# ViV99/slam-experiments

Hardware: AMD Instinct MI355X
Metric: descriptor pairs/sec BF-Hamming knn=2 @64kx64k (higher is better)
Workload: dtype u32

## Files before the change

include/slamhip.h:

```cpp
#ifndef SLAMHIP_H
#define SLAMHIP_H

#include <stdint.h>

#ifdef __cplusplus
extern "C" {
#endif

typedef struct slam_ctx slam_ctx;

#define SLAM_API __attribute__((visibility("default")))

enum slam_status {
    SLAM_OK = 0,
    SLAM_ERR_INVALID = -1,
    SLAM_ERR_HIP = -2,
    SLAM_ERR_NO_DEVICE = -3,
    SLAM_ERR_RCCL = -4,
    SLAM_ERR_STATE = -5,
    SLAM_ERR_BUSY = -6
};

#define SLAM_DESC_BYTES 32
#define SLAM_MAX_TRAIN_PER_PASS (1 << 23)
// ... 29 lines not shown
typedef struct slam_bf_search {
    const void* d_query;
    int64_t N;
    const void* d_train;
    int64_t M;
    int64_t train_base;
    int32_t* d_idx;
    int32_t* d_dist;
} slam_bf_search;
SLAM_API int slam_bf_knn2_batch_u256(slam_ctx* ctx, int64_t B, const slam_bf_search* h_searches);

SLAM_API int slam_bf_merge_top2(slam_ctx* ctx, const int32_t* d_idx_parts,
                       const int32_t* d_dist_parts, int64_t G, int64_t N,
                       int32_t* d_idx, int32_t* d_dist);

SLAM_API int slam_bf_knn2_u256_host(slam_ctx* ctx, const uint8_t* h_query, int64_t N,
                           const uint8_t* h_train, int64_t M,
                           int32_t* h_idx, int32_t* h_dist);

#define SLAM_BF_KNN_MAX 32
SLAM_API int slam_bf_knn_u256(slam_ctx* ctx, const void* d_query, int64_t N, const void* d_train, int64_t M,
                              int64_t train_base, int K, int32_t* d_idx, int32_t* d_dist);
SLAM_API int slam_bf_knn_u256_host(slam_ctx* ctx, const uint8_t* h_query, int64_t N, const uint8_t* h_train, int64_t M,
                                   int K, int32_t* h_idx, int32_t* h_dist);
SLAM_API int slam_bf_merge_topk(slam_ctx* ctx, const int32_t* d_idx_parts, const int32_t* d_dist_parts, int64_t G,
                                int64_t N, int K, int32_t* d_idx, int32_t* d_dist);
SLAM_API int slam_bf_topk_plan_describe(int num_cu, int64_t N, int64_t M, int K, int32_t* h_plan);

SLAM_API int slam_bf_radius_u256(slam_ctx* ctx, const void* d_query, int64_t N, const void* d_train, int64_t M,
                                 float max_distance, int64_t train_base, int64_t* d_offsets, int64_t capacity,
                                 int32_t* d_idx, int32_t* d_dist, int64_t* h_total);
SLAM_API int slam_bf_radius_u256_host(slam_ctx* ctx, const uint8_t* h_query, int64_t N, const uint8_t* h_train, int64_t M,
                                      float max_distance, int64_t* h_offsets, int64_t capacity, int32_t* h_idx,
                                      int32_t* h_dist, int64_t* h_total);
SLAM_API int slam_bf_radius_threshold(float max_distance);
SLAM_API int slam_bf_radius_plan_describe(int num_cu, int64_t N, int64_t M, int32_t* h_plan);

SLAM_API int slam_bf_window_knn_u256(slam_ctx* ctx, const void* d_query, int64_t N, const void* d_train, int64_t M,
                                     const float* d_query_xy, const float* d_train_xy, const float* d_radius, float radius,
                                     int k, int64_t cells, int32_t* d_idx, int32_t* d_dist);
SLAM_API int slam_bf_window_knn_u256_host(slam_ctx* ctx, const uint8_t* h_query, int64_t N, const uint8_t* h_train, int64_t M,
                                          const float* h_query_xy, const float* h_train_xy, const float* h_radius,
                                          float radius, int k, int64_t cells, int32_t* h_idx, int32_t* h_dist);
SLAM_API int slam_bf_window_plan_describe(int num_cu, int64_t N, int64_t M, int64_t cells, int64_t* h_plan);

#define SLAM_BF_KNOBS 10
SLAM_API int slam_bf_set_tuning(slam_ctx* ctx, const int32_t* h_knobs, int count);
SLAM_API int slam_bf_plan_info(slam_ctx* ctx, int64_t N, int64_t M, int32_t* h_plan);
SLAM_API int slam_bf_plan_describe(int num_cu, const int32_t* h_knobs, int count, int64_t N, int64_t M, int64_t qb_all,
                                   int rows_on_host, int32_t* h_plan, int32_t* h_tbl, int64_t tbl_cap, int64_t* tbl_len);
SLAM_API int slam_bf_set_engine(slam_ctx* ctx, int engine);
SLAM_API int slam_bf_mx_plan_describe(int num_cu, int64_t N, int64_t M, int32_t* h_plan, int32_t* h_tbl, int64_t tbl_cap,
                                      int64_t* tbl_len);
SLAM_API int slam_bf_reset_state(slam_ctx* ctx);
SLAM_API int slam_bf_state_dirty(slam_ctx* ctx, int64_t* h_words);

SLAM_API int slam_bf_knn2_select_u256(slam_ctx* ctx, const void* d_query, int64_t N, const void* d_train, int64_t M,
                                      int64_t train_base, int32_t* d_idx, int32_t* d_dist, int mode, double param,
                                      uint8_t* d_keep, int64_t* h_count);

SLAM_API int slam_bf_match_filter(slam_ctx* ctx, const int32_t* d_idx, const int32_t* d_dist,
                         int64_t N, int mode, double param,
                         uint8_t* d_keep, int64_t* h_count, int32_t* h_min_dist);

SLAM_API int slam_bf_cross_check(slam_ctx* ctx, const int32_t* d_fwd_idx, const int32_t* d_fwd_dist, int64_t N,
                        const int32_t* d_rev_idx, int64_t M, int32_t* d_out_idx, int32_t* d_out_dist,
                        int64_t* h_count);

SLAM_API int slam_bf_split_index(slam_ctx* ctx, const int32_t* d_global_idx, int64_t count, const int32_t* d_offsets,
                                 int64_t images, int32_t* d_img_idx, int32_t* d_train_idx);

SLAM_API int slam_reproj_rj_f64(slam_ctx* ctx, const double* d_poses, int64_t K,
                       const double* d_points, int64_t L,
                       const int32_t* d_obs_pose, const int32_t* d_obs_point,
                       const double* d_meas, int64_t O,
                       double fx, double fy, double cx, double cy,
                       double* d_e, double* d_Jpose, double* d_Jpoint);

SLAM_API int slam_index_errors(slam_ctx* ctx, int64_t* count);

SLAM_API int slam_pose_normal_eq_f64(slam_ctx* ctx, const double* d_pose,
                            const double* d_points, const double* d_meas,
                            const uint8_t* d_active, int64_t O,
                            double fx, double fy, double cx, double cy,
                            double huber_delta,
                            double* d_H, double* d_b, double* d_chi2);

SLAM_API int slam_pose_optimize_f64(slam_ctx* ctx, const double* d_pose_in, const double* d_points,
                                    const double* d_meas, int64_t O, double fx, double fy, double cx, double cy,
                                    int rounds, int iterations, double chi2_threshold, double huber_delta,
                                    double* d_pose_out, uint8_t* d_inlier, double* d_chi2, int32_t* d_stats);

SLAM_API int slam_pose_optimize_batch_f64(slam_ctx* ctx, int64_t B, const double* d_pose_in, const double* d_points,
                                          const double* d_meas, const int32_t* d_offsets, int64_t O_total, double fx,
                                          double fy, double cx, double cy, int rounds, int iterations,
                                          double chi2_threshold, double huber_delta, double* d_pose_out,
                                          uint8_t* d_inlier, double* d_chi2, int32_t* d_stats);


SLAM_API int slam_tv_fivepoint_f64(slam_ctx* ctx, int64_t S, const double* d_x1, const double* d_x2, double* d_E,
                                   int32_t* d_nroots);

SLAM_API int slam_tv_essential_ransac_f64(slam_ctx* ctx, int64_t B, const int32_t* d_offsets, const double* d_px1,
                                          const double* d_px2, int64_t M, double fx, double fy, double cx, double cy,
                                          int H, double threshold_px, uint64_t seed, double* d_E, uint8_t* d_inlier,
                                          int32_t* d_stats);
// ... 219 lines not shown
```

slam-experiments_amd/csrc/bf_mx.hip:

```cpp
#include "internal.h"
#include <vector>
#include <atomic>
#include <type_traits>

#include "bf_common.h"

#define SLAM_MX_STAGE 128
#define SLAM_MX_BOUND_LIMIT 0x7F000000u
#define SLAM_MX_EARLY 0x16u
#define SLAM_MX_UNROLL 4
#define SLAM_MX_RESIDENT 4

#ifdef SLAM_MX_PROBE
__device__ unsigned long long* g_mx_probe = nullptr;
extern "C" __attribute__((visibility("default"))) int slam_exp_set_mx_probe(void* p) {
    return (int)hipMemcpyToSymbol(HIP_SYMBOL(g_mx_probe), &p, sizeof(p));
}
#define MX_STAMP(ph) do { const unsigned long long now_ = __builtin_readcyclecounter(); pacc[ph] += now_ - plast; plast = now_; } while (0)
#else
#define MX_STAMP(ph) do {} while (0)
#endif

typedef int mx_v8i __attribute__((ext_vector_type(8)));
typedef float mx_v4f __attribute__((ext_vector_type(4)));

__device__ __forceinline__ uint4 mx_expand(u32 x) {
    uint4 r;
    r.x = ((x << 3) & 0x88888888u) | 0x22222222u;
    r.y = ((x << 2) & 0x88888888u) | 0x22222222u;
    r.z = ((x << 1) & 0x88888888u) | 0x22222222u;
    r.w = (x & 0x88888888u) | 0x22222222u;
    return r;
}

__device__ __forceinline__ mx_v4f mx_dot(uint4 a, uint4 b, mx_v4f c) {
    const mx_v8i av = {(int)a.x, (int)a.y, (int)a.z, (int)a.w, 0, 0, 0, 0};
    const mx_v8i bv = {(int)b.x, (int)b.y, (int)b.z, (int)b.w, 0, 0, 0, 0};
    return __builtin_amdgcn_mfma_scale_f32_16x16x128_f8f6f4(av, bv, c, 4, 4, 0, 127, 0, 127);
}

__device__ __forceinline__ void mx_unite(u32& b1, u32& b2, u32 c1, u32 c2) {
    const u32 n2 = min(max(b1, c1), min(b2, c2));
    b1 = min(b1, c1);
    b2 = n2;
}

__device__ __forceinline__ u32 mx_pick(const u32 (&v)[4], int i) {
    return i == 0 ? v[0] : (i == 1 ? v[1] : (i == 2 ? v[2] : v[3]));
}

__global__ __launch_bounds__(256) __attribute__((amdgpu_waves_per_eu(4, 4))) void bf_top2_mx_kernel(const uint4* __restrict__ q, int N, const uint4* __restrict__ t,
                                                         const int* __restrict__ tbl, bf_state st, int train_base,
                                                         int2* __restrict__ out_idx, int2* __restrict__ out_dist,
                                                         uint4* __restrict__ keep, int nchunks, bf_select sel) {
    __shared__ uint4 tile[2][SLAM_MX_STAGE * 8];
    __shared__ u32 s_ticket, s_last;
    const int tid = threadIdx.x;
    const int lane = tid & 63, wave = tid >> 6;
    const int kg = lane >> 4, col = lane & 15;
#ifdef SLAM_MX_PROBE
    unsigned long long pacc[8] = {0, 0, 0, 0, 0, 0, 0, 0}, plast = __builtin_readcyclecounter();
#endif
    const u32 lanek = (u32)(4 * kg - (1 << SLAM_KEY_IDX_BITS));
    const int bx = ((int)blockIdx.x + (int)blockIdx.y) % (int)gridDim.x;
    auto lane_query = [&]() -> int {
        int v = tid;
        asm volatile("" : "+v"(v));
        return bx * 256 + v;
    };

    uint4 qb[4][2];
    const u32* qw = (const u32*)q;
#pragma unroll
    for (int tt = 0; tt < 4; tt++) {
        int qi = bx * 256 + wave * 64 + tt * 16 + col;
        qi = qi < N ? qi : N - 1;
#pragma unroll
        for (int h = 0; h < 2; h++) qb[tt][h] = mx_expand(qw[(size_t)qi * 8 + h * 4 + kg]);
    }
    if (const int qbase = lane_query(); keep && blockIdx.y == 0 && qbase < N) {
        keep[2 * (size_t)qbase] = q[2 * (size_t)qbase];
        keep[2 * (size_t)qbase + 1] = q[2 * (size_t)qbase + 1];
    }

    u32 b1[4], b2[4];
    mx_v4f cth[4];
    auto set_threshold = [&](int tt, u32 x) {
        const float c = (float)(2 * (int)x - 258);
        cth[tt] = mx_v4f{c, c, c, c};
    };
    auto threshold_x = [&](int tt) -> u32 { return (u32)((int)cth[tt][0] + 258) >> 1; };
#pragma unroll
    for (int tt = 0; tt < 4; tt++) {
        b1[tt] = b2[tt] = SLAM_KEY_NONE;
        set_threshold(tt, SLAM_KEY_NONE >> SLAM_KEY_IDX_BITS);
    }
    auto unite_tile = [&](int tt, u32& u1, u32& u2) {
        u1 = b1[tt];
        u2 = b2[tt];
#pragma unroll
        for (int off = 16; off <= 32; off <<= 1) {
            const u32 c1 = (u32)__shfl_xor((int)u1, off, 64), c2 = (u32)__shfl_xor((int)u2, off, 64);
            mx_unite(u1, u2, c1, c2);
        }
    };
    auto unite_lanes = [&](u32 (&u1)[4], u32 (&u2)[4]) {
#pragma unroll
        for (int tt = 0; tt < 4; tt++) unite_tile(tt, u1[tt], u2[tt]);
    };
    u32 gkey = SLAM_BOUND_IDLE, pend[1] = {0u};
    auto exchange = [&](int c0) {
        u32 u1[4], u2[4];
        unite_lanes(u1, u2);
        if (const int qbase = lane_query(); qbase < N) {
            const u32 own = mx_pick(u2, kg);
            asm volatile("" ::"v"(pend[0]));
            const u32 g = __hip_atomic_load(&st.bound[qbase], __ATOMIC_RELAXED, __HIP_MEMORY_SCOPE_AGENT);
            if (own < g && own < SLAM_MX_BOUND_LIMIT) pend[0] = atomicMin(&st.bound[qbase], own);
            gkey = g;
        }
#pragma unroll
        for (int tt = 0; tt < 4; tt++) {
            const u32 g = (u32)__shfl((int)gkey, tt * 16 + col, 64);
            const u32 gx = g < SLAM_MX_BOUND_LIMIT ? (g >> SLAM_KEY_IDX_BITS) + ((g & SLAM_KEY_IDX_MASK) < (u32)c0 ? 0u : 1u)
                                                   : SLAM_KEY_NONE >> SLAM_KEY_IDX_BITS;
            set_threshold(tt, min(threshold_x(tt), min(gx, u2[tt] >> SLAM_KEY_IDX_BITS)));
        }
    };

    const int srow = tid >> 1, sh = tid & 1;
    auto load_stage = [&](int s, int c1) -> uint4 {
        const uint4* ts = t + 2 * (size_t)s;
        if (s + SLAM_MX_STAGE <= c1) return ts[(u32)tid];
        return s + srow < c1 ? ts[(u32)tid] : make_uint4(0, 0, 0, 0);
    };
    const u32 fill = 0x22222222u;
    auto expand = [&](u32 v) -> uint4 {
        uint4 r;
        asm("v_and_or_b32 %0, %1, %2, %3" : "=v"(r.x) : "v"(v << 3), "s"(0x88888888u), "v"(fill));
        asm("v_and_or_b32 %0, %1, %2, %3" : "=v"(r.y) : "v"(v << 2), "s"(0x88888888u), "v"(fill));
        asm("v_and_or_b32 %0, %1, %2, %3" : "=v"(r.z) : "v"(v << 1), "s"(0x88888888u), "v"(fill));
        asm("v_and_or_b32 %0, %1, %2, %3" : "=v"(r.w) : "v"(v), "s"(0x88888888u), "v"(fill));
        return r;
    };
    uint4* const dst0 = tile[0] + (srow >> 4) * 128 + sh * 64 + (srow & 15);
    auto store_stage = [&](int b, uint4 v) {
        uint4* dst = dst0 + b * (SLAM_MX_STAGE * 8);
        dst[0] = expand(v.x);
        dst[16] = expand(v.y);
        dst[32] = expand(v.z);
        dst[48] = expand(v.w);
    };

    u32* const cursor = st.cursor + (size_t)(4 * bx) * SLAM_CURSOR_STRIDE;
    if (tid == 0) s_ticket = __hip_atomic_fetch_add(cursor, 1u, __ATOMIC_RELAXED, __HIP_MEMORY_SCOPE_AGENT);
    __syncthreads();
    int ci = __builtin_amdgcn_readfirstlane((int)s_ticket);
    int scanned = 0;
    MX_STAMP(0);
    while (ci < nchunks) {
        const int c0 = tbl[ci], c1 = tbl[ci + 1];
        const uint4 first = load_stage(c0, c1);
        exchange(c0);
        store_stage(0, first);
        __syncthreads();
        MX_STAMP(1);
        int buf = 0;
        for (int s0 = c0; s0 < c1; s0 += SLAM_MX_STAGE) {
            const int s1 = s0 + SLAM_MX_STAGE;
            const bool more = s1 < c1;
            if (!more && tid == 0) s_ticket = __hip_atomic_fetch_add(cursor, 1u, __ATOMIC_RELAXED, __HIP_MEMORY_SCOPE_AGENT);
            MX_STAMP(7);
            const int ng = __builtin_amdgcn_readfirstlane(min(SLAM_MX_STAGE / 16, (c1 - s0 + 15) >> 4));
            const uint4* tp = tile[buf];
            u32 fired = 0;
            auto dots0 = [&](const uint4& a, mx_v4f (&acc)[4]) {
#pragma unroll
                for (int tt = 0; tt < 4; tt++) acc[tt] = mx_dot(a, qb[tt][0], cth[tt]);
            };
            auto fold = [&](int g, mx_v4f (&acc)[4], auto rag) {
                int p[4];
#pragma unroll
                for (int tt = 0; tt < 4; tt++)
                    p[tt] = max(max(__float_as_int(acc[tt][0]), __float_as_int(acc[tt][1])), __float_as_int(acc[tt][2]));
                int m = max(max(p[0], __float_as_int(acc[0][3])), p[1]);
                m = max(max(m, __float_as_int(acc[1][3])), p[2]);
                m = max(max(m, __float_as_int(acc[2][3])), p[3]);
                m = max(m, __float_as_int(acc[3][3]));
                if (__builtin_expect(__ballot(m >= 0) != 0ull, 0)) {
                    MX_STAMP(2);
                    int row0 = s0 + g * 16;
                    asm("" : "+s"(row0));
                    const u32 rowk = (u32)row0 + lanek;
#pragma unroll
                    for (int tt = 0; tt < 4; tt++) {
                        if (__ballot(max(p[tt], __float_as_int(acc[tt][3])) >= 0) == 0ull) continue;
                        fired |= 1u << tt;
// ... 116 lines not shown


struct bf_mx_plan {
    int qblocks;
    int workers;
    int chunk;
    int S;
    int tail;
};

static bf_mx_plan make_mx_plan_core(int num_cu, int resident, int64_t N, int64_t M, std::vector<int>* tbl) {
    bf_mx_plan p;
    p.qblocks = (int)((N + 255) / 256);
    int64_t W = (int64_t)num_cu * resident / p.qblocks;
    if (W < 1) W = 1;
    if (W > 256) W = 256;
    const int64_t c = M / W >= 8192 ? 1024 : 256;
    std::vector<int>& b = *tbl;
    b.clear();
    b.push_back(0);
    int shrinking = 0;
    for (int64_t at = 0; at < M;) {
        int64_t len = c;
        const int64_t g = (M - at) / (2 * W) / SLAM_MX_STAGE * SLAM_MX_STAGE;
        if (g < len) { len = g < SLAM_MX_STAGE ? SLAM_MX_STAGE : g; shrinking++; }
        at = at + len < M ? at + len : M;
        b.push_back((int)at);
    }
    p.chunk = (int)c;
    p.S = (int)b.size() - 1;
    p.tail = shrinking;
    p.workers = (int)(W < p.S ? W : p.S);
    return p;
}

static bool bf_mx_auto(int64_t N, int64_t M) {
    return (N >= 8192 && M >= 16384) || (N >= 3000 && M >= 40000) || (N >= 1000 && M >= 65536) || (N >= 500 && M >= 200000);
}

extern "C" int slam_bf_mx_plan_describe(int num_cu, int64_t N, int64_t M, int32_t* h_plan, int32_t* h_tbl, int64_t tbl_cap,
                                        int64_t* tbl_len) {
    SLAM_REQUIRE(num_cu >= 1 && num_cu <= 4096, "num_cu out of range");
    SLAM_REQUIRE(N >= 1 && M >= 1 && M <= SLAM_MAX_TRAIN_PER_PASS && N <= (1ll << 30), "bad sizes");
    SLAM_REQUIRE(h_plan && tbl_len && (h_tbl || tbl_cap == 0) && tbl_cap >= 0, "slam_bf_mx_plan_describe: null argument");
    std::vector<int> tbl;
    const bf_mx_plan p = make_mx_plan_core(num_cu, SLAM_MX_RESIDENT, N, M, &tbl);
    h_plan[0] = p.qblocks; h_plan[1] = p.workers; h_plan[2] = p.chunk; h_plan[3] = p.S;
    h_plan[4] = p.tail; h_plan[5] = SLAM_MX_STAGE; h_plan[6] = SLAM_MX_RESIDENT; h_plan[7] = bf_mx_auto(N, M) ? 1 : 0;
    *tbl_len = (int64_t)tbl.size();
    for (int64_t i = 0; i < (int64_t)tbl.size() && i < tbl_cap; i++) h_tbl[i] = tbl[(size_t)i];
    return SLAM_OK;
}

extern "C" int slam_bf_set_engine(slam_ctx* ctx, int engine) {
    SLAM_REQUIRE(ctx, "slam_bf_set_engine: null ctx");
    SLAM_REQUIRE(engine >= 0 && engine <= 2, "engine must be 0 (auto), 1 (VALU) or 2 (matrix cores where eligible)");
    std::lock_guard<std::mutex> g(ctx->mu);
    ctx->bf_engine = engine;
    return SLAM_OK;
}

bool bf_mx_route(slam_ctx* ctx, int64_t N, int64_t M, bool rows_on_host) {
    std::lock_guard<std::mutex> g(ctx->mu);
    if (ctx->bf_engine == 1 || rows_on_host) return false;
    for (int i = 0; i < SLAM_BF_KNOBS; i++)
        if (ctx->bf_knob[i]) return false;
    return ctx->bf_engine == 2 || bf_mx_auto(N, M);
}

int bf_mx_pass(slam_ctx* ctx, const void* d_query, int64_t N, const void* d_train, int64_t M, int64_t train_base, int32_t* d_idx,
               int32_t* d_dist, void* d_keep, const bf_select& sel, int* qblocks_out) {
    static std::atomic<int> occ_once{0};
    int occ = occ_once.load(std::memory_order_relaxed);
    if (!occ) {
        int o = 0;
        SLAM_HIP(hipOccupancyMaxActiveBlocksPerMultiprocessor(&o, bf_top2_mx_kernel, 256, 0));
        occ = o > 0 ? o : SLAM_MX_RESIDENT;
        occ_once.store(occ, std::memory_order_relaxed);
    }
    std::vector<int> tbl;
    int num_cu;
    {
        std::lock_guard<std::mutex> g(ctx->mu);
        num_cu = ctx->num_cu;
    }
    const bf_mx_plan p = make_mx_plan_core(num_cu, occ, N, M, &tbl);
    bf_state st;
    if (int rc = bf_state_get(ctx, N, &st)) return rc;
    const int* d_tbl = nullptr;
    if (int rc = bf_table_get(ctx, tbl, &d_tbl)) return rc;
    if (qblocks_out) *qblocks_out = p.qblocks;
    SLAM_HIP(hipGetLastError());
    if (int rc = slam_prof_begin(ctx)) return rc;
    bf_top2_mx_kernel<<<dim3(p.qblocks, p.workers), dim3(256), 0, ctx->stream>>>(
        (const uint4*)d_query, (int)N, (const uint4*)d_train, d_tbl, st, (int)train_base, (int2*)d_idx, (int2*)d_dist,
        (uint4*)d_keep, p.S, sel);
    if (int rc = slam_prof_end(ctx)) return rc;
    const hipError_t e = hipGetLastError();
    if (e != hipSuccess) {
        (void)bf_state_reset(ctx);
        return slam_set_error(SLAM_ERR_HIP, "top-2 MX kernel launch failed: %s", hipGetErrorString(e));
    }
    return SLAM_OK;
}
```

slam-experiments_amd/slamhip/__init__.py:

```python
from ._lib import NO_MATCH_DIST, NO_MATCH_IDX, SlamHipBusy, SlamHipError, device_count, load
from .device import Context, DeviceBuffer, default_context, mx_plan_describe, plan_describe
from .matching import (
    NORM_HAMMING,
    DeviceDescriptors,
    KeyframeDatabase,
    ResidentMatcher,
    Top2Table,
    as_descriptors,
    check_topk_k,
    cross_check_arrays,
    knn2_device,
    knn2_device_batch,
    knn2_select_device,
    knn_match_arrays,
    knn_match_arrays_batch,
    knn_match_collection,
    knn_topk_device,
    match_arrays,
    plan_describe_radius,
    plan_describe_topk,
    plan_describe_window,
    radius_device,
    radius_match_arrays,
    radius_match_collection,
    radius_threshold,
    ratio_test_arrays,
    split_image_index,
    topk_match_arrays,
    topk_match_collection,
    window_knn_device,
    window_match_arrays,
    window_match_filtered,
)
from .homography import (
    decompose_homography_arrays,
    decompose_homography_batch,
    decompose_homography_offsets,
    estimate_two_view_auto,
    find_homography_arrays,
    find_homography_batch,
    find_homography_offsets,
    fourpoint_homography_arrays,
    model_scores_offsets,
    verify_pairs_auto,
)
from .orb import (
    OrbExtractor,
    OrbFeatureDetector,
    OrbParams,
    OrbResult,
    orb_extract_arrays,
)
from .pnp import (
    loop_edges_from_pnp,
# ... 50 lines not shown
```

slam-experiments_amd/slamhip/_lib.py:

```python
from __future__ import annotations

import ctypes
import os
from ctypes import POINTER, c_char_p, c_double, c_float, c_int, c_int32, c_int64, c_uint8, c_uint64, c_void_p

_HERE = os.path.dirname(os.path.abspath(__file__))
LIB_PATH = os.path.join(os.path.dirname(_HERE), "lib", "libslamhip.so")

SLAM_OK = 0
NO_MATCH_IDX = -1
NO_MATCH_DIST = 2**31 - 1
DESC_BYTES = 32
COMM_ID_BYTES = 128
P2P_HANDLE_BYTES = 64


class SlamHipError(RuntimeError):

    def __init__(self, code: int, message: str):
        super().__init__(f"libslamhip error {code}: {message}")
        self.code = code


class SlamHipBusy(SlamHipError):
    """SLAM_ERR_BUSY (-6): a resource condition, not a caller error - a kernel that needs all its workgroups resident at once
    could not get them (other work holds compute units).  Inputs and outputs are untouched; retry, or use the form without
    a residency requirement."""


SLAM_ERR_INVALID, SLAM_ERR_BUSY = -1, -6


SIGNATURES = {
    "slam_last_error": (c_char_p, []),
    "slam_version": (c_char_p, []),
    "slam_device_count": (c_int, [POINTER(c_int)]),
    "slam_ctx_create": (c_int, [c_int, POINTER(c_void_p)]),
    "slam_ctx_destroy": (c_int, [c_void_p]),
    "slam_ctx_device": (c_int, [c_void_p, POINTER(c_int)]),
    "slam_sync": (c_int, [c_void_p]),
    "slam_malloc": (c_int, [c_void_p, c_uint64, POINTER(c_void_p)]),
    "slam_free": (c_int, [c_void_p, c_void_p]),
    "slam_memset": (c_int, [c_void_p, c_void_p, c_int, c_uint64]),
    "slam_copy": (c_int, [c_void_p, c_void_p, c_void_p, c_uint64]),
    "slam_upload": (c_int, [c_void_p, c_void_p, c_void_p, c_uint64]),
    "slam_download": (c_int, [c_void_p, c_void_p, c_void_p, c_uint64]),
    "slam_timer_start": (c_int, [c_void_p]),
    "slam_timer_stop": (c_int, [c_void_p, POINTER(c_float)]),
    "slam_prof_enable": (c_int, [c_void_p, c_int]),
    "slam_prof_read": (c_int, [c_void_p, POINTER(c_int64), POINTER(c_double)]),
    "slam_bf_knn2_u256": (c_int, [c_void_p, c_void_p, c_int64, c_void_p, c_int64, c_int64, c_void_p, c_void_p]),
    "slam_bf_knn2_batch_u256": (c_int, [c_void_p, c_int64, c_void_p]),
    "slam_bf_knn2_select_u256": (c_int, [c_void_p, c_void_p, c_int64, c_void_p, c_int64, c_int64, c_void_p, c_void_p, c_int, c_double,
                                         c_void_p, POINTER(c_int64)]),
    "slam_bf_merge_top2": (c_int, [c_void_p, c_void_p, c_void_p, c_int64, c_int64, c_void_p, c_void_p]),
    "slam_bf_knn2_u256_host": (c_int, [c_void_p, c_void_p, c_int64, c_void_p, c_int64, c_void_p, c_void_p]),
    "slam_bf_knn_u256": (c_int, [c_void_p, c_void_p, c_int64, c_void_p, c_int64, c_int64, c_int, c_void_p, c_void_p]),
    "slam_bf_knn_u256_host": (c_int, [c_void_p, c_void_p, c_int64, c_void_p, c_int64, c_int, c_void_p, c_void_p]),
    "slam_bf_merge_topk": (c_int, [c_void_p, c_void_p, c_void_p, c_int64, c_int64, c_int, c_void_p, c_void_p]),
    "slam_bf_topk_plan_describe": (c_int, [c_int, c_int64, c_int64, c_int, POINTER(c_int32)]),
    "slam_bf_radius_u256": (c_int, [c_void_p, c_void_p, c_int64, c_void_p, c_int64, c_float, c_int64, c_void_p, c_int64, c_void_p,
                                    c_void_p, POINTER(c_int64)]),
    "slam_bf_radius_u256_host": (c_int, [c_void_p, c_void_p, c_int64, c_void_p, c_int64, c_float, c_void_p, c_int64, c_void_p,
                                         c_void_p, POINTER(c_int64)]),
    "slam_bf_radius_threshold": (c_int, [c_float]),
    "slam_bf_radius_plan_describe": (c_int, [c_int, c_int64, c_int64, POINTER(c_int32)]),
    "slam_bf_window_knn_u256": (c_int, [c_void_p, c_void_p, c_int64, c_void_p, c_int64, c_void_p, c_void_p, c_void_p, c_float,
                                        c_int, c_int64, c_void_p, c_void_p]),
    "slam_bf_window_knn_u256_host": (c_int, [c_void_p, c_void_p, c_int64, c_void_p, c_int64, c_void_p, c_void_p, c_void_p,
                                             c_float, c_int, c_int64, c_void_p, c_void_p]),
    "slam_bf_window_plan_describe": (c_int, [c_int, c_int64, c_int64, c_int64, POINTER(c_int64)]),
    "slam_bf_set_tuning": (c_int, [c_void_p, POINTER(c_int32), c_int]),
    "slam_bf_plan_info": (c_int, [c_void_p, c_int64, c_int64, POINTER(c_int32)]),
    "slam_bf_plan_describe": (c_int, [c_int, POINTER(c_int32), c_int, c_int64, c_int64, c_int64, c_int, POINTER(c_int32),
                                      POINTER(c_int32), c_int64, POINTER(c_int64)]),
    "slam_bf_set_engine": (c_int, [c_void_p, c_int]),
    "slam_bf_mx_plan_describe": (c_int, [c_int, c_int64, c_int64, POINTER(c_int32), POINTER(c_int32), c_int64, POINTER(c_int64)]),
    "slam_bf_reset_state": (c_int, [c_void_p]),
    "slam_bf_state_dirty": (c_int, [c_void_p, POINTER(c_int64)]),
    "slam_bf_match_filter": (c_int, [c_void_p, c_void_p, c_void_p, c_int64, c_int, c_double, c_void_p,
                                     POINTER(c_int64), POINTER(c_int32)]),
    "slam_bf_cross_check": (c_int, [c_void_p, c_void_p, c_void_p, c_int64, c_void_p, c_int64, c_void_p, c_void_p,
                                    POINTER(c_int64)]),
    "slam_bf_split_index": (c_int, [c_void_p, c_void_p, c_int64, c_void_p, c_int64, c_void_p, c_void_p]),
    "slam_reproj_rj_f64": (c_int, [c_void_p, c_void_p, c_int64, c_void_p, c_int64, c_void_p, c_void_p, c_void_p,
                                   c_int64, c_double, c_double, c_double, c_double, c_void_p, c_void_p, c_void_p]),
    "slam_pose_normal_eq_f64": (c_int, [c_void_p, c_void_p, c_void_p, c_void_p, c_void_p, c_int64, c_double,
                                        c_double, c_double, c_double, c_double, c_void_p, c_void_p, c_void_p]),
    "slam_pose_optimize_f64": (c_int, [c_void_p, c_void_p, c_void_p, c_void_p, c_int64, c_double, c_double, c_double,
                                       c_double, c_int, c_int, c_double, c_double, c_void_p, c_void_p, c_void_p,
                                       c_void_p]),
    "slam_pose_optimize_batch_f64": (c_int, [c_void_p, c_int64, c_void_p, c_void_p, c_void_p, c_void_p, c_int64, c_double,
                                             c_double, c_double, c_double, c_int, c_int, c_double, c_double, c_void_p,
                                             c_void_p, c_void_p, c_void_p]),
    "slam_tv_fivepoint_f64": (c_int, [c_void_p, c_int64, c_void_p, c_void_p, c_void_p, c_void_p]),
    "slam_tv_essential_ransac_f64": (c_int, [c_void_p, c_int64, c_void_p, c_void_p, c_void_p, c_int64, c_double, c_double, c_double,
                                             c_double, c_int, c_double, c_uint64, c_void_p, c_void_p, c_void_p]),
    "slam_tv_recover_pose_f64": (c_int, [c_void_p, c_int64, c_void_p, c_void_p, c_void_p, c_int64, c_double, c_double, c_double,
                                         c_double, c_void_p, c_void_p, c_double, c_void_p, c_void_p, c_void_p]),
    "slam_tv_triangulate_f64": (c_int, [c_void_p, c_int64, c_void_p, c_void_p, c_void_p, c_void_p, c_void_p, c_void_p]),
    "slam_pnp_p3p_f64": (c_int, [c_void_p, c_int64, c_void_p, c_void_p, c_void_p, c_void_p]),
    "slam_pnp_ransac_f64": (c_int, [c_void_p, c_int64, c_void_p, c_void_p, c_void_p, c_int64, c_double, c_double, c_double, c_double,
                                    c_int, c_double, c_uint64, c_void_p, c_void_p, c_void_p]),
    "slam_hg_fourpoint_f64": (c_int, [c_void_p, c_int64, c_void_p, c_void_p, c_void_p, c_void_p]),
    "slam_hg_ransac_f64": (c_int, [c_void_p, c_int64, c_void_p, c_void_p, c_void_p, c_int64, c_int, c_double, c_uint64, c_void_p,
                                   c_void_p, c_void_p]),
    "slam_hg_decompose_f64": (c_int, [c_void_p, c_int64, c_void_p, c_void_p, c_void_p, c_int64, c_double, c_double, c_double, c_double,
                                      c_void_p, c_void_p, c_double, c_void_p, c_void_p, c_void_p, c_void_p, c_void_p, c_void_p,
                                      c_void_p]),
    "slam_hg_model_score_f64": (c_int, [c_void_p, c_int64, c_void_p, c_void_p, c_void_p, c_int64, c_double, c_double, c_double,
                                        c_double, c_void_p, c_void_p, c_double, c_void_p, c_void_p]),
    "slam_sim3_threepoint_f64": (c_int, [c_void_p, c_int64, c_void_p, c_void_p, c_int, c_void_p, c_void_p]),
    "slam_sim3_ransac_f64": (c_int, [c_void_p, c_int64, c_void_p, c_void_p, c_void_p, c_int64, c_void_p, c_double, c_double, c_double,
                                     c_double, c_int, c_double, c_int, c_uint64, c_void_p, c_void_p, c_void_p]),
    "slam_sim3_refit_f64": (c_int, [c_void_p, c_int64, c_void_p, c_void_p, c_void_p, c_int64, c_void_p, c_int, c_void_p, c_void_p]),
    "slam_pg_workspace": (c_int, [c_int64, c_int64, POINTER(c_uint64)]),
    "slam_pg_plan": (c_int, [c_int64, c_int64, POINTER(c_int32)]),
    "slam_pg_linearize_f64": (c_int, [c_void_p, c_int64, c_int64, c_void_p, c_void_p, c_void_p, c_void_p, c_void_p, c_void_p,
                                      c_double, c_void_p, c_void_p, c_void_p, c_void_p, POINTER(c_int32)]),
    "slam_pg_hmul_f64": (c_int, [c_void_p, c_int64, c_int64, c_void_p, c_void_p, c_void_p, c_void_p, c_void_p, c_void_p,
                                 c_double, c_void_p, c_void_p]),
    "slam_pg_pcg_f64": (c_int, [c_void_p, c_int64, c_int64, c_void_p, c_void_p, c_void_p, c_void_p, c_void_p, c_void_p,
                                c_void_p, c_double, c_double, c_int, c_void_p, c_void_p]),
    "slam_pg_optimize_f64": (c_int, [c_void_p, c_int64, c_int64, c_void_p, c_void_p, c_void_p, c_void_p, c_void_p, c_int64,
                                     c_void_p, c_void_p, c_int, c_double, c_double, c_int, c_void_p, c_void_p]),
    "slam_pg_optimize_host_f64": (c_int, [c_void_p, c_int64, c_int64, c_void_p, c_void_p, c_void_p, c_void_p, c_void_p, c_int,
                                          c_double, c_double, c_int, c_void_p, c_void_p]),
    "slam_s3g_workspace": (c_int, [c_int64, c_int64, POINTER(c_uint64)]),
    "slam_s3g_plan": (c_int, [c_int64, c_int64, POINTER(c_int32)]),
    "slam_s3g_linearize_f64": (c_int, [c_void_p, c_int64, c_int64, c_void_p, c_void_p, c_void_p, c_void_p, c_void_p, c_void_p,
# ... 106 lines not shown
```

slam-experiments_amd/slamhip/device.py:

```python
from __future__ import annotations

import ctypes
import threading
from typing import Optional, Tuple

import numpy as np

from . import _lib
from ._lib import check


class DeviceBuffer:

    __slots__ = ("ctx", "ptr", "nbytes", "_owner")

    def __init__(self, ctx: "Context", ptr: int, nbytes: int, owner: Optional["DeviceBuffer"] = None):
        self.ctx = ctx
        self.ptr = ptr
        self.nbytes = nbytes
        self._owner = owner

    def view(self, offset: int, nbytes: Optional[int] = None) -> "DeviceBuffer":
        nbytes = self.nbytes - offset if nbytes is None else nbytes
        if offset < 0 or nbytes < 0 or offset + nbytes > self.nbytes:
# ... 71 lines not shown

    def plan_info(self, n: int, m: int) -> dict:
        p = (ctypes.c_int32 * 10)()
        check(self.lib.slam_bf_plan_info(self.handle, n, m, p))
        return dict(zip(("R", "qblocks", "chunk", "chunks", "lead_rows", "lead_chunks", "tail_chunks", "cus", "sgpr_feed", "cold_rows"), p))

    def sync(self) -> None:
        check(self.lib.slam_sync(self.handle))

    def timer_start(self) -> None:
        check(self.lib.slam_timer_start(self.handle))

    def timer_stop(self) -> float:
        ms = ctypes.c_float(0)
        check(self.lib.slam_timer_stop(self.handle, ctypes.byref(ms)))
        return ms.value

    def prof_enable(self, on: bool = True) -> None:
        check(self.lib.slam_prof_enable(self.handle, int(on)))

    def prof_read(self) -> Tuple[int, float]:
        n = ctypes.c_int64(0)
        ms = ctypes.c_double(0)
        check(self.lib.slam_prof_read(self.handle, ctypes.byref(n), ctypes.byref(ms)))
        return n.value, ms.value


_default_lock = threading.Lock()
_default_ctx: Optional[Context] = None


def default_context() -> Context:
    global _default_ctx
    with _default_lock:
        if _default_ctx is None:
            _default_ctx = Context(0)
        return _default_ctx


PLAN_KNOBS = ("R", "blocks_per_cu", "lead_rows", "lead_chunk", "tail", "feed", "cold", "chunk", "queue", "merge")


def mx_plan_describe(n: int, m: int, num_cu: int = 256):
    lib = _lib.load()
    plan = (ctypes.c_int32 * 8)()
    cap = 1 << 16
    tbl = (ctypes.c_int32 * cap)()
    length = ctypes.c_int64(0)
    check(lib.slam_bf_mx_plan_describe(num_cu, n, m, plan, tbl, cap, ctypes.byref(length)))
    names = ("qblocks", "workers", "chunk", "chunks", "tail_chunks", "stage_rows", "resident", "auto")
    return dict(zip(names, plan)), list(tbl[:min(length.value, cap)])


def plan_describe(n: int, m: int, num_cu: int = 256, qb_all: int = 0, rows_on_host: bool = False, **knobs):
    unknown = set(knobs) - set(PLAN_KNOBS)
    if unknown:
        raise TypeError(f"unknown knobs {sorted(unknown)}")
    lib = _lib.load()
    k = (ctypes.c_int32 * len(PLAN_KNOBS))(*(int(knobs.get(name, 0)) for name in PLAN_KNOBS))
    plan = (ctypes.c_int32 * 14)()
    cap = 1 << 16
    tbl = (ctypes.c_int32 * cap)()
    length = ctypes.c_int64(0)
    check(lib.slam_bf_plan_describe(num_cu, k, len(PLAN_KNOBS), n, m, qb_all, int(rows_on_host), plan, tbl, cap, ctypes.byref(length)))
    names = ("R", "qblocks", "chunk", "chunks", "lead_rows", "lead_chunks", "tail_chunks", "cus", "sgpr_feed", "cold_rows",
             "table_free", "bound_free", "workers", "resident")
    out = dict(zip(names, plan))
    out["merge"], out["resident"] = out["resident"] >> 8, out["resident"] & 255
    return out, list(tbl[:min(length.value, cap)])
```

Measured before the change: 10660 billion.

## Add 32x32x64 MFMA variant of the top-2 Hamming matcher and auto-select it

Adds a new kernel that uses the 32x32x64 scaled f8f6f4 MFMA instead of 16x16x128, so each wave handles two 32-query tiles against 32-row train groups with a matching LDS layout and fold logic. Shared helpers move to a common header. The host picks the 32-wide kernel automatically for N<=131072 and M<=200000, so the 64k x 64k case takes it. The larger MFMA tile is meant to raise the compute per operand load, at the cost of more accumulator registers and a different threshold and fold pattern.

After: 10830 billion (median of 6 runs). +1.6%, better.

```diff
diff --git a/include/slamhip.h b/include/slamhip.h
--- a/include/slamhip.h
+++ b/include/slamhip.h
@@ -105,6 +105,7 @@
 SLAM_API int slam_bf_set_engine(slam_ctx* ctx, int engine);
 SLAM_API int slam_bf_mx_plan_describe(int num_cu, int64_t N, int64_t M, int32_t* h_plan, int32_t* h_tbl, int64_t tbl_cap,
                                       int64_t* tbl_len);
+SLAM_API int slam_bf_mx_tile_describe(int engine, int64_t N, int64_t M, int32_t* h_tile);
 SLAM_API int slam_bf_reset_state(slam_ctx* ctx);
 SLAM_API int slam_bf_state_dirty(slam_ctx* ctx, int64_t* h_words);
 
diff --git a/slam-experiments_amd/csrc/bf_mx.hip b/slam-experiments_amd/csrc/bf_mx.hip
--- a/slam-experiments_amd/csrc/bf_mx.hip
+++ b/slam-experiments_amd/csrc/bf_mx.hip
@@ -4,12 +4,9 @@
 #include <type_traits>
 
 #include "bf_common.h"
-
-#define SLAM_MX_STAGE 128
-#define SLAM_MX_BOUND_LIMIT 0x7F000000u
-#define SLAM_MX_EARLY 0x16u
+#include "bf_mx_common.h"
+
 #define SLAM_MX_UNROLL 4
-#define SLAM_MX_RESIDENT 4
 
 #ifdef SLAM_MX_PROBE
 __device__ unsigned long long* g_mx_probe = nullptr;
@@ -21,28 +18,12 @@
 #define MX_STAMP(ph) do {} while (0)
 #endif
 
-typedef int mx_v8i __attribute__((ext_vector_type(8)));
 typedef float mx_v4f __attribute__((ext_vector_type(4)));
-
-__device__ __forceinline__ uint4 mx_expand(u32 x) {
-    uint4 r;
-    r.x = ((x << 3) & 0x88888888u) | 0x22222222u;
-    r.y = ((x << 2) & 0x88888888u) | 0x22222222u;
-    r.z = ((x << 1) & 0x88888888u) | 0x22222222u;
-    r.w = (x & 0x88888888u) | 0x22222222u;
-    return r;
-}
 
 __device__ __forceinline__ mx_v4f mx_dot(uint4 a, uint4 b, mx_v4f c) {
     const mx_v8i av = {(int)a.x, (int)a.y, (int)a.z, (int)a.w, 0, 0, 0, 0};
     const mx_v8i bv = {(int)b.x, (int)b.y, (int)b.z, (int)b.w, 0, 0, 0, 0};
     return __builtin_amdgcn_mfma_scale_f32_16x16x128_f8f6f4(av, bv, c, 4, 4, 0, 127, 0, 127);
-}
-
-__device__ __forceinline__ void mx_unite(u32& b1, u32& b2, u32 c1, u32 c2) {
-    const u32 n2 = min(max(b1, c1), min(b2, c2));
-    b1 = min(b1, c1);
-    b2 = n2;
 }
 
 __device__ __forceinline__ u32 mx_pick(const u32 (&v)[4], int i) {
@@ -122,8 +103,7 @@
 #pragma unroll
         for (int tt = 0; tt < 4; tt++) {
             const u32 g = (u32)__shfl((int)gkey, tt * 16 + col, 64);
-            const u32 gx = g < SLAM_MX_BOUND_LIMIT ? (g >> SLAM_KEY_IDX_BITS) + ((g & SLAM_KEY_IDX_MASK) < (u32)c0 ? 0u : 1u)
-                                                   : SLAM_KEY_NONE >> SLAM_KEY_IDX_BITS;
+            const u32 gx = mx_bound_x(g, c0);
             set_threshold(tt, min(threshold_x(tt), min(gx, u2[tt] >> SLAM_KEY_IDX_BITS)));
         }
     };
@@ -135,14 +115,7 @@
         return s + srow < c1 ? ts[(u32)tid] : make_uint4(0, 0, 0, 0);
     };
     const u32 fill = 0x22222222u;
-    auto expand = [&](u32 v) -> uint4 {
-        uint4 r;
-        asm("v_and_or_b32 %0, %1, %2, %3" : "=v"(r.x) : "v"(v << 3), "s"(0x88888888u), "v"(fill));
-        asm("v_and_or_b32 %0, %1, %2, %3" : "=v"(r.y) : "v"(v << 2), "s"(0x88888888u), "v"(fill));
-        asm("v_and_or_b32 %0, %1, %2, %3" : "=v"(r.z) : "v"(v << 1), "s"(0x88888888u), "v"(fill));
-        asm("v_and_or_b32 %0, %1, %2, %3" : "=v"(r.w) : "v"(v), "s"(0x88888888u), "v"(fill));
-        return r;
-    };
+    auto expand = [&](u32 v) -> uint4 { return mx_expand_op(v, fill); };
     uint4* const dst0 = tile[0] + (srow >> 4) * 128 + sh * 64 + (srow & 15);
     auto store_stage = [&](int b, uint4 v) {
         uint4* dst = dst0 + b * (SLAM_MX_STAGE * 8);
@@ -365,9 +338,22 @@
     return SLAM_OK;
 }
 
+static bool bf_mx32_auto(int64_t N, int64_t M) {
+    return N <= 131072 && M <= 200000;
+}
+
+extern "C" int slam_bf_mx_tile_describe(int engine, int64_t N, int64_t M, int32_t* h_tile) {
+    SLAM_REQUIRE(h_tile, "slam_bf_mx_tile_describe: null argument");
+    SLAM_REQUIRE(engine == 0 || engine == 2 || engine == 3, "engine must be 0 (auto), 2 or 3");
+    SLAM_REQUIRE(N >= 1 && M >= 1, "bad sizes");
+    *h_tile = engine == 3 || (engine == 0 && bf_mx32_auto(N, M)) ? 32 : 16;
+    return SLAM_OK;
+}
+
 extern "C" int slam_bf_set_engine(slam_ctx* ctx, int engine) {
     SLAM_REQUIRE(ctx, "slam_bf_set_engine: null ctx");
-    SLAM_REQUIRE(engine >= 0 && engine <= 2, "engine must be 0 (auto), 1 (VALU) or 2 (matrix cores where eligible)");
+    SLAM_REQUIRE(engine >= 0 && engine <= 3,
+                 "engine must be 0 (auto), 1 (VALU), 2 (16x16 matrix-core kernel where eligible) or 3 (32x32 matrix-core kernel where eligible)");
     std::lock_guard<std::mutex> g(ctx->mu);
     ctx->bf_engine = engine;
     return SLAM_OK;
@@ -378,25 +364,28 @@
     if (ctx->bf_engine == 1 || rows_on_host) return false;
     for (int i = 0; i < SLAM_BF_KNOBS; i++)
         if (ctx->bf_knob[i]) return false;
-    return ctx->bf_engine == 2 || bf_mx_auto(N, M);
+    return ctx->bf_engine == 2 || ctx->bf_engine == 3 || bf_mx_auto(N, M);
 }
 
 int bf_mx_pass(slam_ctx* ctx, const void* d_query, int64_t N, const void* d_train, int64_t M, int64_t train_base, int32_t* d_idx,
                int32_t* d_dist, void* d_keep, const bf_select& sel, int* qblocks_out) {
-    static std::atomic<int> occ_once{0};
-    int occ = occ_once.load(std::memory_order_relaxed);
-    if (!occ) {
-        int o = 0;
-        SLAM_HIP(hipOccupancyMaxActiveBlocksPerMultiprocessor(&o, bf_top2_mx_kernel, 256, 0));
-        occ = o > 0 ? o : SLAM_MX_RESIDENT;
-        occ_once.store(occ, std::memory_order_relaxed);
-    }
-    std::vector<int> tbl;
-    int num_cu;
+    int num_cu, engine;
     {
         std::lock_guard<std::mutex> g(ctx->mu);
         num_cu = ctx->num_cu;
-    }
+        engine = ctx->bf_engine;
+    }
+    const bool wide = engine == 3 || (engine == 0 && bf_mx32_auto(N, M));
+    const auto kernel = wide ? bf_top2_mx32_kernel : bf_top2_mx_kernel;
+    static std::atomic<int> occ_once[2] = {{0}, {0}};
+    int occ = occ_once[wide].load(std::memory_order_relaxed);
+    if (!occ) {
+        int o = 0;
+        SLAM_HIP(hipOccupancyMaxActiveBlocksPerMultiprocessor(&o, kernel, 256, 0));
+        occ = o > 0 ? o : SLAM_MX_RESIDENT;
+        occ_once[wide].store(occ, std::memory_order_relaxed);
+    }
+    std::vector<int> tbl;
     const bf_mx_plan p = make_mx_plan_core(num_cu, occ, N, M, &tbl);
     bf_state st;
     if (int rc = bf_state_get(ctx, N, &st)) return rc;
@@ -405,7 +394,7 @@
     if (qblocks_out) *qblocks_out = p.qblocks;
     SLAM_HIP(hipGetLastError());
     if (int rc = slam_prof_begin(ctx)) return rc;
-    bf_top2_mx_kernel<<<dim3(p.qblocks, p.workers), dim3(256), 0, ctx->stream>>>(
+    kernel<<<dim3(p.qblocks, p.workers), dim3(256), 0, ctx->stream>>>(
         (const uint4*)d_query, (int)N, (const uint4*)d_train, d_tbl, st, (int)train_base, (int2*)d_idx, (int2*)d_dist,
         (uint4*)d_keep, p.S, sel);
     if (int rc = slam_prof_end(ctx)) return rc;
diff --git a/slam-experiments_amd/csrc/bf_mx32.hip b/slam-experiments_amd/csrc/bf_mx32.hip
--- /dev/null
+++ b/slam-experiments_amd/csrc/bf_mx32.hip
@@ -0,0 +1,221 @@
+#include "internal.h"
+#include <type_traits>
+
+#include "bf_common.h"
+#include "bf_mx_common.h"
+
+typedef float mx_v16f __attribute__((ext_vector_type(16)));
+
+__device__ __forceinline__ mx_v16f mx32_dot(uint4 a, uint4 b, mx_v16f c) {
+    const mx_v8i av = {(int)a.x, (int)a.y, (int)a.z, (int)a.w, 0, 0, 0, 0};
+    const mx_v8i bv = {(int)b.x, (int)b.y, (int)b.z, (int)b.w, 0, 0, 0, 0};
+    return __builtin_amdgcn_mfma_scale_f32_32x32x64_f8f6f4(av, bv, c, 4, 4, 0, 0, 0, 0);
+}
+
+#define MX32_GROUP 32
+#define MX32_GROUPS (SLAM_MX_STAGE / MX32_GROUP)
+
+__global__ __launch_bounds__(256) __attribute__((amdgpu_waves_per_eu(4, 4))) void bf_top2_mx32_kernel(
+    const uint4* __restrict__ q, int N, const uint4* __restrict__ t, const int* __restrict__ tbl, bf_state st, int train_base,
+    int2* __restrict__ out_idx, int2* __restrict__ out_dist, uint4* __restrict__ keep, int nchunks, bf_select sel) {
+    __shared__ uint4 tile[2][SLAM_MX_STAGE * 8];
+    __shared__ u32 s_ticket, s_last;
+    const int tid = threadIdx.x;
+    const int lane = tid & 63, wave = tid >> 6;
+    const int hk = lane >> 5, col = lane & 31;
+    const int bx = ((int)blockIdx.x + (int)blockIdx.y) % (int)gridDim.x;
+    auto lane_query = [&]() -> int {
+        int v = tid;
+        asm volatile("" : "+v"(v));
+        return bx * 256 + v;
+    };
+
+    uint4 qb[2][4];
+    const u32* qw = (const u32*)q;
+#pragma unroll
+    for (int tt = 0; tt < 2; tt++) {
+        int qi = bx * 256 + wave * 64 + tt * 32 + col;
+        qi = qi < N ? qi : N - 1;
+#pragma unroll
+        for (int kq = 0; kq < 4; kq++) qb[tt][kq] = mx_expand(qw[(size_t)qi * 8 + kq * 2 + hk]);
+    }
+    if (const int qbase = lane_query(); keep && blockIdx.y == 0 && qbase < N) {
+        keep[2 * (size_t)qbase] = q[2 * (size_t)qbase];
+        keep[2 * (size_t)qbase + 1] = q[2 * (size_t)qbase + 1];
+    }
+
+    u32 b1[2], b2[2], xs[2];
+    int thr[2];
+    auto set_threshold = [&](int tt, u32 x) {
+        xs[tt] = x;
+        thr[tt] = x > 129u ? (int)0x80000000u : __float_as_int((float)(258 - 2 * (int)x));
+    };
+#pragma unroll
+    for (int tt = 0; tt < 2; tt++) {
+        b1[tt] = b2[tt] = SLAM_KEY_NONE;
+        set_threshold(tt, SLAM_KEY_NONE >> SLAM_KEY_IDX_BITS);
+    }
+    auto unite_tile = [&](int tt, u32& u1, u32& u2) {
+        u1 = b1[tt];
+        u2 = b2[tt];
+        const u32 c1 = (u32)__shfl_xor((int)u1, 32, 64), c2 = (u32)__shfl_xor((int)u2, 32, 64);
+        mx_unite(u1, u2, c1, c2);
+    };
+    u32 gkey = SLAM_BOUND_IDLE, pend[1] = {0u};
+    auto exchange = [&](int c0) {
+        u32 u1[2], u2[2];
+#pragma unroll
+        for (int tt = 0; tt < 2; tt++) unite_tile(tt, u1[tt], u2[tt]);
+        if (const int qbase = lane_query(); qbase < N) {
+            const u32 own = hk ? u2[1] : u2[0];
+            asm volatile("" ::"v"(pend[0]));
+            const u32 g = __hip_atomic_load(&st.bound[qbase], __ATOMIC_RELAXED, __HIP_MEMORY_SCOPE_AGENT);
+            if (own < g && own < SLAM_MX_BOUND_LIMIT) pend[0] = atomicMin(&st.bound[qbase], own);
+            gkey = g;
+        }
+#pragma unroll
+        for (int tt = 0; tt < 2; tt++) {
+            const u32 g = (u32)__shfl((int)gkey, tt * 32 + col, 64);
+            set_threshold(tt, min(xs[tt], min(mx_bound_x(g, c0), u2[tt] >> SLAM_KEY_IDX_BITS)));
+        }
+    };
+
+    const int srow = tid >> 1, sh = tid & 1;
+    auto load_stage = [&](int s, int c1) -> uint4 {
+        const uint4* ts = t + 2 * (size_t)s;
+        if (s + SLAM_MX_STAGE <= c1) return ts[(u32)tid];
+        return s + srow < c1 ? ts[(u32)tid] : make_uint4(0, 0, 0, 0);
+    };
+    const u32 fill = 0x22222222u;
+    uint4* const dst0 = tile[0] + (srow >> 5) * 256 + sh * 128 + (srow & 31);
+    auto store_word = [&](uint4* dst, int j, u32 v) { dst[(j >> 1) * 64 + (j & 1) * 32] = mx_expand_op(v, fill); };
+    auto store_stage = [&](int b, uint4 v) {
+        uint4* dst = dst0 + b * (SLAM_MX_STAGE * 8);
+        store_word(dst, 0, v.x);
+        store_word(dst, 1, v.y);
+        store_word(dst, 2, v.z);
+        store_word(dst, 3, v.w);
+    };
+
+    u32* const cursor = st.cursor + (size_t)(4 * bx) * SLAM_CURSOR_STRIDE;
+    if (tid == 0) s_ticket = __hip_atomic_fetch_add(cursor, 1u, __ATOMIC_RELAXED, __HIP_MEMORY_SCOPE_AGENT);
+    __syncthreads();
+    int ci = __builtin_amdgcn_readfirstlane((int)s_ticket);
+    int scanned = 0;
+    while (ci < nchunks) {
+        const int c0 = tbl[ci], c1 = tbl[ci + 1];
+        const uint4 first = load_stage(c0, c1);
+        exchange(c0);
+        store_stage(0, first);
+        __syncthreads();
+        int buf = 0;
+        for (int s0 = c0; s0 < c1; s0 += SLAM_MX_STAGE) {
+            const int s1 = s0 + SLAM_MX_STAGE;
+            const bool more = s1 < c1;
+            if (!more && tid == 0) s_ticket = __hip_atomic_fetch_add(cursor, 1u, __ATOMIC_RELAXED, __HIP_MEMORY_SCOPE_AGENT);
+            const uint4* tp = tile[buf];
+            u32 fired = 0;
+            auto fold = [&](int g, const mx_v16f (&acc)[2], auto rag) {
+                int m[2];
+#pragma unroll
+                for (int tt = 0; tt < 2; tt++) {
+                    int p = max(max(__float_as_int(acc[tt][0]), __float_as_int(acc[tt][1])), __float_as_int(acc[tt][2]));
+#pragma unroll
+                    for (int i = 3; i < 15; i += 2) p = max(max(p, __float_as_int(acc[tt][i])), __float_as_int(acc[tt][i + 1]));
+                    m[tt] = max(p, __float_as_int(acc[tt][15]));
+                }
+                if (__builtin_expect(__ballot(m[0] >= thr[0] || m[1] >= thr[1]) != 0ull, 0)) {
+                    int row0 = s0 + g * MX32_GROUP;
+                    asm("" : "+s"(row0));
+                    const u32 rowk = (u32)row0 + (u32)(4 * hk);
+#pragma unroll
+                    for (int tt = 0; tt < 2; tt++) {
+                        if (__ballot(m[tt] >= thr[tt]) == 0ull) continue;
+                        fired |= 1u << tt;
+                        const u32 base = (128u << SLAM_KEY_IDX_BITS) + rowk;
+#pragma unroll
+                        for (int i = 0; i < 16; i++) {
+                            if (__ballot(__float_as_int(acc[tt][i]) >= thr[tt]) == 0ull) continue;
+                            const int off = 8 * (i >> 2) + (i & 3);
+                            u32 key = base + (u32)off + ((u32)(int)(-acc[tt][i]) << (SLAM_KEY_IDX_BITS - 1));
+                            if constexpr (decltype(rag)::value)
+                                key = (int)rowk + off < c1 ? key : SLAM_KEY_NONE;
+                            b2[tt] = umed3(b1[tt], b2[tt], key);
+                            b1[tt] = min(b1[tt], key);
+                        }
+                        set_threshold(tt, min(xs[tt], b2[tt] >> SLAM_KEY_IDX_BITS));
+                    }
+                }
+            };
+            const mx_v16f zero = {0, 0, 0, 0, 0, 0, 0, 0, 0, 0, 0, 0, 0, 0, 0, 0};
+            auto group = [&](int g, auto rag) {
+                mx_v16f acc[2];
+#pragma unroll
+                for (int kq = 0; kq < 4; kq++) {
+                    const uint4 a = tp[g * 256 + kq * 64 + lane];
+#pragma unroll
+                    for (int tt = 0; tt < 2; tt++) acc[tt] = mx32_dot(a, qb[tt][kq], kq ? acc[tt] : zero);
+                }
+                fold(g, acc, rag);
+            };
+            auto trip = [&](auto shadow) {
+                constexpr bool SH = decltype(shadow)::value;
+                const uint4* ap = tp + lane;
+                uint4* const dst = dst0 + (buf ^ 1) * (SLAM_MX_STAGE * 8);
+                u32 nx[4] = {0, 0, 0, 0};
+                if (SH) {
+                    const uint4 x = (t + 2 * (size_t)s1)[2 * min(srow, c1 - 1 - s1) + sh];
+                    nx[0] = x.x; nx[1] = x.y; nx[2] = x.z; nx[3] = x.w;
+                }
+                uint4 a[4];
+#pragma unroll
+                for (int kq = 0; kq < 4; kq++) a[kq] = ap[kq * 64];
+#pragma unroll
+                for (int k = 0; k < MX32_GROUPS; k++) {
+                    mx_v16f acc[2];
+#pragma unroll
+                    for (int kq = 0; kq < 4; kq++) {
+                        __builtin_amdgcn_sched_barrier(0);
+#pragma unroll
+                        for (int tt = 0; tt < 2; tt++) acc[tt] = mx32_dot(a[kq], qb[tt][kq], kq ? acc[tt] : zero);
+                        __builtin_amdgcn_sched_barrier(0);
+                        if (k + 1 < MX32_GROUPS) a[kq] = ap[(k + 1) * 256 + kq * 64];
+                        if (SH && k >= 1 && kq == 1) store_word(dst, k - 1, nx[k - 1]);
+                        if (SH && k == 3 && kq == 2) store_word(dst, 3, nx[3]);
+                    }
+                    __builtin_amdgcn_sched_barrier(0);
+                    fold(k, acc, std::false_type{});
+                    __builtin_amdgcn_sched_barrier(0);
+                }
+            };
+            if (more) {
+                trip(std::true_type{});
+            } else if (s1 == c1) {
+                trip(std::false_type{});
+            } else {
+                const int ng = __builtin_amdgcn_readfirstlane((c1 - s0 + MX32_GROUP - 1) / MX32_GROUP);
+                for (int g = 0; g < ng; g++) group(g, std::true_type{});
+            }
+#pragma unroll
+            for (int tt = 0; tt < 2; tt++) {
+                if (!(fired >> tt & 1u)) continue;
+                u32 u1, u2;
+                unite_tile(tt, u1, u2);
+                set_threshold(tt, min(xs[tt], u2 >> SLAM_KEY_IDX_BITS));
+            }
+            scanned += min(s1, c1) - s0;
+            if (more && scanned < 32 * SLAM_MX_STAGE && (SLAM_MX_EARLY >> (scanned / SLAM_MX_STAGE) & 1u)) exchange(s1);
+            __syncthreads();
+            buf ^= 1;
+        }
+        ci = __builtin_amdgcn_readfirstlane((int)s_ticket);
+    }
+
+    u32 u1[2], u2[2];
+#pragma unroll
+    for (int tt = 0; tt < 2; tt++) unite_tile(tt, u1[tt], u2[tt]);
+    const u32 f1[1] = {hk ? u1[1] : u1[0]}, f2[1] = {hk ? u2[1] : u2[0]};
+    const u32 gk[1] = {gkey < SLAM_MX_BOUND_LIMIT ? gkey >> SLAM_KEY_IDX_BITS : SLAM_BOUND_IDLE};
+    bf_top2_epilogue<1, true>(st, bx, tid, lane, lane_query(), false, false, f1, f2, gk, pend, N, (int)gridDim.y, train_base, out_idx,
+                              out_dist, sel, s_last);
+}
diff --git a/slam-experiments_amd/csrc/bf_mx_common.h b/slam-experiments_amd/csrc/bf_mx_common.h
--- /dev/null
+++ b/slam-experiments_amd/csrc/bf_mx_common.h
@@ -0,0 +1,43 @@
+#pragma once
+#include "internal.h"
+#include "bf_common.h"
+
+#define SLAM_MX_STAGE 128
+#define SLAM_MX_BOUND_LIMIT 0x7F000000u
+#define SLAM_MX_EARLY 0x16u
+#define SLAM_MX_RESIDENT 4
+
+typedef int mx_v8i __attribute__((ext_vector_type(8)));
+
+__device__ __forceinline__ uint4 mx_expand(u32 x) {
+    uint4 r;
+    r.x = ((x << 3) & 0x88888888u) | 0x22222222u;
+    r.y = ((x << 2) & 0x88888888u) | 0x22222222u;
+    r.z = ((x << 1) & 0x88888888u) | 0x22222222u;
+    r.w = (x & 0x88888888u) | 0x22222222u;
+    return r;
+}
+
+__device__ __forceinline__ uint4 mx_expand_op(u32 v, u32 fill) {
+    uint4 r;
+    asm("v_and_or_b32 %0, %1, %2, %3" : "=v"(r.x) : "v"(v << 3), "s"(0x88888888u), "v"(fill));
+    asm("v_and_or_b32 %0, %1, %2, %3" : "=v"(r.y) : "v"(v << 2), "s"(0x88888888u), "v"(fill));
+    asm("v_and_or_b32 %0, %1, %2, %3" : "=v"(r.z) : "v"(v << 1), "s"(0x88888888u), "v"(fill));
+    asm("v_and_or_b32 %0, %1, %2, %3" : "=v"(r.w) : "v"(v), "s"(0x88888888u), "v"(fill));
+    return r;
+}
+
+__device__ __forceinline__ void mx_unite(u32& b1, u32& b2, u32 c1, u32 c2) {
+    const u32 n2 = min(max(b1, c1), min(b2, c2));
+    b1 = min(b1, c1);
+    b2 = n2;
+}
+
+__device__ __forceinline__ u32 mx_bound_x(u32 g, int c0) {
+    return g < SLAM_MX_BOUND_LIMIT ? (g >> SLAM_KEY_IDX_BITS) + ((g & SLAM_KEY_IDX_MASK) < (u32)c0 ? 0u : 1u)
+                                   : SLAM_KEY_NONE >> SLAM_KEY_IDX_BITS;
+}
+
+__global__ void bf_top2_mx32_kernel(const uint4* __restrict__ q, int N, const uint4* __restrict__ t, const int* __restrict__ tbl,
+                                    bf_state st, int train_base, int2* __restrict__ out_idx, int2* __restrict__ out_dist,
+                                    uint4* __restrict__ keep, int nchunks, bf_select sel);
diff --git a/slam-experiments_amd/slamhip/__init__.py b/slam-experiments_amd/slamhip/__init__.py
--- a/slam-experiments_amd/slamhip/__init__.py
+++ b/slam-experiments_amd/slamhip/__init__.py
@@ -1,5 +1,5 @@
 from ._lib import NO_MATCH_DIST, NO_MATCH_IDX, SlamHipBusy, SlamHipError, device_count, load
-from .device import Context, DeviceBuffer, default_context, mx_plan_describe, plan_describe
+from .device import Context, DeviceBuffer, default_context, mx_plan_describe, mx_tile_describe, plan_describe
 from .matching import (
     NORM_HAMMING,
     DeviceDescriptors,
diff --git a/slam-experiments_amd/slamhip/_lib.py b/slam-experiments_amd/slamhip/_lib.py
--- a/slam-experiments_amd/slamhip/_lib.py
+++ b/slam-experiments_amd/slamhip/_lib.py
@@ -76,6 +76,7 @@
                                       POINTER(c_int32), c_int64, POINTER(c_int64)]),
     "slam_bf_set_engine": (c_int, [c_void_p, c_int]),
     "slam_bf_mx_plan_describe": (c_int, [c_int, c_int64, c_int64, POINTER(c_int32), POINTER(c_int32), c_int64, POINTER(c_int64)]),
+    "slam_bf_mx_tile_describe": (c_int, [c_int, c_int64, c_int64, POINTER(c_int32)]),
     "slam_bf_reset_state": (c_int, [c_void_p]),
     "slam_bf_state_dirty": (c_int, [c_void_p, POINTER(c_int64)]),
     "slam_bf_match_filter": (c_int, [c_void_p, c_void_p, c_void_p, c_int64, c_int, c_double, c_void_p,
diff --git a/slam-experiments_amd/slamhip/device.py b/slam-experiments_amd/slamhip/device.py
--- a/slam-experiments_amd/slamhip/device.py
+++ b/slam-experiments_amd/slamhip/device.py
@@ -147,6 +147,12 @@
     return dict(zip(names, plan)), list(tbl[:min(length.value, cap)])
 
 
+def mx_tile_describe(n: int, m: int, engine: int = 0) -> int:
+    tile = ctypes.c_int32(0)
+    check(_lib.load().slam_bf_mx_tile_describe(int(engine), n, m, ctypes.byref(tile)))
+    return tile.value
+
+
 def plan_describe(n: int, m: int, num_cu: int = 256, qb_all: int = 0, rows_on_host: bool = False, **knobs):
     unknown = set(knobs) - set(PLAN_KNOBS)
     if unknown:
```
